# HanielUlises/GCN-GrabCut

Measured on AMD Instinct MI355X. Metric: images/sec end-to-end mask (DUTS-shape batch), higher is better.
Workload: dtype f32

## Files before the change

### gcn-grabcut_amd/csrc/ggc_maxflow.hip

```cpp
#include "ggc_gc.h"
#include "ggc_mf_sweep.h"
#include "ggc_mf_push.h"
#include <algorithm>
#include <chrono>
#include <cstdlib>
#include <vector>

namespace ggc {

constexpr int RT = MF_RT;
constexpr int PT_W = MF_PT_W, PT_H = MF_PT_H;
constexpr int PT_N = PT_W * PT_H;
constexpr int PUSH_GRID = 1024, RELAX_GRID = 1024, ASYNC_GRID = 128;

__global__ void __launch_bounds__(256) k_mf_zero3(int32_t* __restrict__ a, size_t na, int32_t* __restrict__ b, size_t nb, int32_t* __restrict__ c, size_t nc) {
    const size_t i = (size_t)blockIdx.x * 256 + threadIdx.x;
    if (i < na) a[i] = 0;
    else if (i < na + nb) b[i - na] = 0;
    else if (i < na + nb + nc) c[i - na - nb] = 0;
}
void mf_zero3(hipStream_t st, int32_t* a, size_t na, int32_t* b, size_t nb, int32_t* c, size_t nc) {
    const size_t n = na + nb + nc;
    if (n) hipLaunchKernelGGL(k_mf_zero3, dim3(cdiv(n, 256)), dim3(256), 0, st, a, na, b, nb, c, nc);
}

__device__ __forceinline__ void aq_zero(unsigned long long* __restrict__ ring, int32_t* __restrict__ q, int cap) {
    const size_t n_thr = (size_t)gridDim.x * gridDim.y * blockDim.x;
    const size_t i0 = ((size_t)blockIdx.y * gridDim.x + blockIdx.x) * blockDim.x + threadIdx.x;
    for (size_t i = i0; i < (size_t)cap; i += n_thr) ring[i] = 0ull;
    if (i0 < (size_t)AQ_WORDS) q[i0] = 0;
}

constexpr int OUT_CAP = 1024;
struct OutList { int n, base; int buf[OUT_CAP]; };
__device__ __forceinline__ void push_tile_l(int tile, int32_t* __restrict__ flag, OutList& L, int32_t* __restrict__ list,
                                            int32_t* __restrict__ count) {
    if (ldg(&flag[tile]) == 0 && atomicExch(&flag[tile], 1) == 0) {
        const int i = atomicAdd(&L.n, 1);
        if (i < OUT_CAP) L.buf[i] = tile;
        else list[atomicAdd(count, 1)] = tile;
    }
}
__device__ __forceinline__ void flush_tiles(OutList& L, int32_t* __restrict__ list, int32_t* __restrict__ count) {
    __syncthreads();
    const int n = min(L.n, OUT_CAP);
    if (threadIdx.x == 0 && n > 0) L.base = atomicAdd(count, n);
    __syncthreads();
    for (int i = threadIdx.x; i < n; i += blockDim.x) list[L.base + i] = L.buf[i];
}

__global__ void __launch_bounds__(256) k_mf_rinit(GcDims d, MfTiles tl, const int32_t* __restrict__ open_list,
                                                  const int32_t* __restrict__ snk, int32_t* __restrict__ dist,
                                                  int32_t* __restrict__ list, int32_t* __restrict__ flag, int32_t* __restrict__ flag2,
                                                  int32_t* __restrict__ count, int32_t* __restrict__ active, int32_t* __restrict__ scan,
                                                  unsigned long long* __restrict__ ring, int32_t* __restrict__ q, int cap) {
    constexpr int T = MF_RT;
    __shared__ OutList outl;
    if (threadIdx.x == 0) outl.n = 0;
    aq_zero(ring, q, cap);
    if (blockIdx.x == 0 && threadIdx.x == 0) active[open_list[blockIdx.y]] = 0;
    if (blockIdx.x == 0 && blockIdx.y == 0 && threadIdx.x < 8 && (threadIdx.x == 0 || threadIdx.x >= 4)) scan[threadIdx.x] = 0;
    __syncthreads();
    const int tiles_per_image = tl.rt_x * tl.rt_y;
    const int tr = blockIdx.x * 4 + (threadIdx.x >> 6), lane = threadIdx.x & 63;
    if (tr < tiles_per_image) {
        const int b = open_list[blockIdx.y];
        const int ty0 = (tr / tl.rt_x) * T, tx0 = (tr % tl.rt_x) * T;
        const int lx = lane & 31, h = lane >> 5;
        const size_t base = (size_t)b * d.P;
        int sv[16];
#pragma unroll
        for (int r = 0; r < 16; ++r) sv[r] = snk[base + (size_t)min(ty0 + 16 * h + r, d.H - 1) * d.W + min(tx0 + lx, d.W - 1)];
        bool open_px = false;
#pragma unroll
        for (int r = 0; r < 16; ++r) {
            const int y = ty0 + 16 * h + r, x = tx0 + lx;
            if (x < d.W && y < d.H) {
                dist[base + (size_t)y * d.W + x] = sv[r] > 0 ? 1 : DINF;
                open_px |= sv[r] <= 0;
            }
        }
        const bool listed = __any(open_px);
        if (lane == 0) {
            const int tile = b * tiles_per_image + tr;
            flag[tile] = listed ? 1 : 0;
            flag2[tile] = 0;
            if (listed) {
                const int i = atomicAdd(&outl.n, 1);
                if (i < OUT_CAP) outl.buf[i] = tile; else list[atomicAdd(count, 1)] = tile;
            }
        }
    }
    flush_tiles(outl, list, count);
}

template <bool PROF>
__global__ void __launch_bounds__(256) k_mf_relax_wave(GcDims d, MfTiles tl, int phase, long long* __restrict__ prof, uint8_t* __restrict__ rmask,
                                                       int32_t* __restrict__ dirty, const int32_t* __restrict__ rc, int32_t* __restrict__ dist, int32_t* __restrict__ counters,
                                                       const int32_t* __restrict__ list_in, int32_t* __restrict__ list_out,
                                                       int32_t* __restrict__ flag_in, int32_t* __restrict__ flag_out) {
    __shared__ RelaxWaveLds lds[4];
    __shared__ OutList outl;
    if (threadIdx.x == 0) outl.n = 0;
    __syncthreads();
    const int wv = threadIdx.x >> 6;
    const int n_in = counters[phase % 3];
    int32_t* n_out = counters + (phase + 1) % 3;
    if (blockIdx.x == 0 && threadIdx.x == 0) counters[(phase + 2) % 3] = 0;
    const int tiles_per_image = tl.rt_x * tl.rt_y;
    const int G = gridDim.x * 4;
    MfRelaxClocks<PROF> ck;
    int tile_nx = blockIdx.x * 4 + wv < n_in ? list_in[blockIdx.x * 4 + wv] : 0;
    for (int t = blockIdx.x * 4 + wv; t < n_in; t += G) {
        int lane = threadIdx.x & 63;
        asm volatile("" : "+v"(lane));
        ck.begin();
        const int tile = __builtin_amdgcn_readfirstlane(tile_nx);
        tile_nx = t + G < n_in ? list_in[t + G] : 0;
        const int nbm = mf_relax_visit<false, PROF, GGC_MF_RELAX_BFS != 0>(d, tl, tile, lane, lds[wv], rmask, dirty, rc, dist, flag_in, ck);
        const int b = tile / tiles_per_image, tr = tile % tiles_per_image;
        const int tyi = tr / tl.rt_x, txi = tr % tl.rt_x;
        if (lane < 9 && (nbm >> lane) & 1) {
            const int ty = tyi + lane / 3 - 1, tx = txi + lane % 3 - 1;
            if (ty >= 0 && ty < tl.rt_y && tx >= 0 && tx < tl.rt_x)
                push_tile_l(b * tiles_per_image + ty * tl.rt_x + tx, flag_out, outl, list_out, n_out);
        }
        mf_wave_sync();
        ck.end();
    }
    if (PROF && (threadIdx.x & 63) == 0 && ck.sum[3]) {
        unsigned long long* q = reinterpret_cast<unsigned long long*>(prof) + (64 + (blockIdx.x & 63)) * 8;
        for (int k = 0; k < 7; ++k) atomicAdd(&q[k], (unsigned long long)ck.sum[k]);
    }
    flush_tiles(outl, list_out, n_out);
}

#ifndef GGC_MF_PUSH_WAVE
#define GGC_MF_PUSH_WAVE 1
#endif
constexpr int PUSH_WAVE_GRID_DIV = 2;
template <bool PROF>
__global__ void __launch_bounds__(256) k_mf_pr_wave(GcDims d, MfTiles tl, int phase, int inner, long long* __restrict__ prof,
                                                    int32_t* __restrict__ rc, int32_t* __restrict__ ex,
                                                    int32_t* __restrict__ snk, int32_t* __restrict__ dist, uint8_t* __restrict__ rmask,
                                                    int32_t* __restrict__ dirty, int32_t* __restrict__ counters, const int32_t* __restrict__ list_in,
                                                    int32_t* __restrict__ list_out, int32_t* __restrict__ flag_in,
                                                    int32_t* __restrict__ flag_out) {
    __shared__ PushTileLds<PT_H> lds[4];
    __shared__ OutList outl;
    if (threadIdx.x == 0) outl.n = 0;
    __syncthreads();
    const int wv = threadIdx.x >> 6;
    const int n_in = counters[phase % 3];
    int32_t* n_out = counters + (phase + 1) % 3;
    if (blockIdx.x == 0 && threadIdx.x == 0) counters[(phase + 2) % 3] = 0;
    const int tiles_per_image = tl.pt_x * tl.pt_y;
    const size_t BP = (size_t)d.B * d.P;
    const int G = gridDim.x * 4;
    long long pv[4] = {0, 0, 0, 0}, p_all = 0, p_n = 0;
    int tile_nx = blockIdx.x * 4 + wv < n_in ? list_in[blockIdx.x * 4 + wv] : 0;
    for (int t = blockIdx.x * 4 + wv; t < n_in; t += G) {
        int lane = threadIdx.x & 63;
        asm volatile("" : "+v"(lane));
        const long long t_0 = PROF ? wall_clock64() : 0;
        const int tile = __builtin_amdgcn_readfirstlane(tile_nx);
        tile_nx = t + G < n_in ? list_in[t + G] : 0;
        const int b = tile / tiles_per_image, tr = tile % tiles_per_image;
        const int tyi = tr / tl.pt_x, txi = tr % tl.pt_x;
        if (lane == 0) flag_in[tile] = 0;
        const int nbm = push_tile_visit<PT_H, false>(d, tyi, txi, inner, (size_t)b * d.P, BP, rc, ex, snk, dist, rmask, lds[wv], lane, PROF, pv);
        if (lane < 9 && (nbm >> lane) & 1) {
            const int ty = tyi + lane / 3 - 1, tx = txi + lane % 3 - 1;
            if (ty >= 0 && ty < tl.pt_y && tx >= 0 && tx < tl.pt_x) {
                const int nbt = b * tiles_per_image + ty * tl.pt_x + tx;
                if (lane != 4) dirty[nbt] = 1;
                push_tile_l(nbt, flag_out, outl, list_out, n_out);
            }
        }
        mf_wave_sync();
        if (PROF) { p_all += wall_clock64() - t_0; ++p_n; }
    }
    if (PROF && (threadIdx.x & 63) == 0 && p_n) {
        unsigned long long* o = reinterpret_cast<unsigned long long*>(prof) + (192 + (blockIdx.x & 63)) * 8;
        atomicAdd(&o[0], (unsigned long long)pv[0]); atomicAdd(&o[1], (unsigned long long)pv[1]);
        atomicAdd(&o[2], (unsigned long long)(p_all - pv[0] - pv[1]));
        atomicAdd(&o[3], (unsigned long long)p_n); atomicAdd(&o[4], (unsigned long long)pv[2]); atomicAdd(&o[5], (unsigned long long)pv[3]);
    }
    flush_tiles(outl, list_out, n_out);
}

#if !GGC_MF_PUSH_WAVE
__global__ void __launch_bounds__(PT_N) k_mf_pr_list(GcDims d, MfTiles tl, int phase, int inner,
                                                    int32_t* __restrict__ rc, int32_t* __restrict__ ex,
                                                    int32_t* __restrict__ snk, int32_t* __restrict__ dist, uint8_t* __restrict__ rmask,
                                                    int32_t* __restrict__ dirty, int32_t* __restrict__ counters, const int32_t* __restrict__ list_in,
                                                    int32_t* __restrict__ list_out, int32_t* __restrict__ flag_in,
                                                    int32_t* __restrict__ flag_out) {
    __shared__ int s_ex[PT_N];
    __shared__ int s_d[PT_H + 2][PT_W + 2];
    __shared__ int s_rc[8][PT_N];
    __shared__ OutList outl;
    __shared__ int s_nbm;
    const int tid = threadIdx.x, lx = tid & 31;
    if (tid == 0) outl.n = 0;
    const int n_in = counters[phase % 3];
    int32_t* n_out = counters + (phase + 1) % 3;
    if (blockIdx.x == 0 && tid == 0) counters[(phase + 2) % 3] = 0;
    const int tiles_per_image = tl.pt_x * tl.pt_y;
    const size_t BP = (size_t)d.B * d.P;
    constexpr int N_HALO = (PT_H + 2) * (PT_W + 2), HALO_IT = (N_HALO + PT_N - 1) / PT_N;
    struct TileRegs { int e, sk, r[8], hv[HALO_IT]; };
    auto load_tile = [&](int tile, TileRegs& R) {
        const int b = tile / tiles_per_image, tr = tile % tiles_per_image;
        const int tyi = tr / tl.pt_x, txi = tr % tl.pt_x;
        const int x = txi * PT_W + lx;
        const size_t base = (size_t)b * d.P;
        const int y = tyi * PT_H + (tid >> 5);
        const bool in = x < d.W && y < d.H;
        const int p = y * d.W + x;
        R.e = in ? ex[base + p] : 0;
        R.sk = in ? snk[base + p] : 0;
#pragma unroll
        for (int dir = 0; dir < 8; ++dir) R.r[dir] = in ? rc[rc_idx(dir, base + p)] : 0;
#pragma unroll
        for (int k = 0; k < HALO_IT; ++k) {
            const int i = tid + k * PT_N;
            const int gy = tyi * PT_H + i / (PT_W + 2) - 1, gx = txi * PT_W + i % (PT_W + 2) - 1;
            R.hv[k] = (i < N_HALO && gx >= 0 && gx < d.W && gy >= 0 && gy < d.H) ? dist[base + (size_t)gy * d.W + gx] : DINF;
        }
    };
    const int G = gridDim.x;
    int t = blockIdx.x;
    if (t >= n_in) return;
    int tile_next = list_in[t];
    int tile_next2 = t + G < n_in ? list_in[t + G] : 0;
    TileRegs N;
    load_tile(tile_next, N);
    for (; t < n_in; t += G) {
        const int tile = tile_next;
        const int b = tile / tiles_per_image, tr = tile % tiles_per_image;
        const int tyi = tr / tl.pt_x, txi = tr % tl.pt_x;
        const int x = txi * PT_W + lx;
        const size_t base = (size_t)b * d.P;
        __syncthreads();
        const int y = tyi * PT_H + (tid >> 5);
        const bool inb = x < d.W && y < d.H;
        const int pp = y * d.W + x;
        const int e0 = N.e, sk0 = N.sk;
        int sk = sk0, r0[8];
        s_ex[tid] = e0;
#pragma unroll
        for (int dir = 0; dir < 8; ++dir) { r0[dir] = N.r[dir]; s_rc[dir][tid] = r0[dir]; }
#pragma unroll
        for (int k = 0; k < HALO_IT; ++k) {
            const int i = tid + k * PT_N;
            if (i < N_HALO) s_d[i / (PT_W + 2)][i % (PT_W + 2)] = N.hv[k];
        }
        if (t + G < n_in) {
            tile_next = tile_next2;
            tile_next2 = t + 2 * G < n_in ? list_in[t + 2 * G] : 0;
            load_tile(tile_next, N);
        }
        __syncthreads();
        if (tid == 0) { flag_in[tile] = 0; s_nbm = 0; }
        const int d0 = s_d[(tid >> 5) + 1][lx + 1];
        int nbm = 0;
        for (int it = 0; it < inner; ++it) {
            int act = 0;
            if (inb) {
                const int slot = tid, ly = slot >> 5;
                const int e = __hip_atomic_load(&s_ex[slot], __ATOMIC_RELAXED, __HIP_MEMORY_SCOPE_WORKGROUP);
                const int dp = s_d[ly + 1][lx + 1];
                if (e > 0 && dp < d.P) {
                    act = 1;
                    int r[8], hq[8];
#pragma unroll
                    for (int dir = 0; dir < 8; ++dir) {
                        r[dir] = __hip_atomic_load(&s_rc[dir][slot], __ATOMIC_RELAXED, __HIP_MEMORY_SCOPE_WORKGROUP);
                        hq[dir] = s_d[ly + 1 + dir_dy(dir)][lx + 1 + dir_dx(dir)];
                    }
                    int hmin = sk > 0 ? 0 : DINF, best = sk > 0 ? 8 : -1, rb = 0;
#pragma unroll
                    for (int dir = 0; dir < 8; ++dir) {
                        const bool ok = r[dir] > 0 && hq[dir] < hmin;
                        hmin = ok ? hq[dir] : hmin; best = ok ? dir : best; rb = ok ? r[dir] : rb;
                    }
                    if (best >= 0 && dp > hmin) {
                        if (best == 8) {
                            const int dl = min(e, sk);
                            sk -= dl;
                            atomicSub(&s_ex[slot], dl);
                        } else {
                            const int dl = min(e, rb);
                            atomicSub(&s_rc[best][slot], dl);
                            atomicSub(&s_ex[slot], dl);
                            const int bx = dir_dx(best), by = dir_dy(best);
                            const int qlx = lx + bx, qly = ly + by;
                            if (qlx >= 0 && qlx < PT_W && qly >= 0 && qly < PT_H) {
                                const int qt = qly * PT_W + qlx;
                                atomicAdd(&s_rc[best ^ 1][qt], dl);
                                atomicAdd(&s_ex[qt], dl);
                            } else {
                                const int q = pp + by * d.W + bx;
                                atomicAdd(&rc[rc_idx((best ^ 1), base + q)], dl);
                                atomicAdd(&ex[base + q], dl);
                                const int tdy = qly < 0 ? -1 : (qly >= PT_H ? 1 : 0), tdx = qlx < 0 ? -1 : (qlx >= PT_W ? 1 : 0);
                                nbm |= 1 << ((tdy + 1) * 3 + tdx + 1);
                            }
                        }
                    } else {
                        s_d[ly + 1][lx + 1] = (best >= 0 && hmin < DINF) ? hmin + 1 : DINF;
                    }
                }
            }
            if (!__syncthreads_or(act)) break;
        }
        int left = 0;
        if (inb) {
            const int slot = tid, ly = slot >> 5, p = pp;
            const bool ring = lx == 0 || lx == PT_W - 1 || ly == 0 || ly == PT_H - 1;
            const int e1 = s_ex[slot];
            if (e1 != e0) { if (ring) atomicAdd(&ex[base + p], e1 - e0); else ex[base + p] = e1; }
            int m1 = 0, chg = 0;
#pragma unroll
            for (int dir = 0; dir < 8; ++dir) {
                const int r1 = s_rc[dir][slot];
                m1 |= (r1 > 0) ? (1 << dir) : 0;
                if (r1 != r0[dir]) {
                    chg = 1;
                    const bool out = (ly == 0 && dir_dy(dir) < 0) || (ly == PT_H - 1 && dir_dy(dir) > 0) ||
                                     (lx == 0 && dir_dx(dir) < 0) || (lx == PT_W - 1 && dir_dx(dir) > 0);
                    if (out) atomicAdd(&rc[rc_idx(dir, base + p)], r1 - r0[dir]);
                    else rc[rc_idx(dir, base + p)] = r1;
                }
// ... 286 lines not shown
```

### gcn-grabcut_amd/csrc/ggc_maxflow_async.hip

```cpp
#include "ggc_gc.h"
#include "ggc_mf_sweep.h"
#include "ggc_mf_push.h"
#include <algorithm>
#include <cstdlib>

namespace ggc {
namespace {

constexpr int PT_H = MF_PT_H;
constexpr long long AQ_TIMEOUT = 200000000ll;

__device__ __forceinline__ unsigned long long ldg64(const unsigned long long* p) { return __hip_atomic_load(p, __ATOMIC_RELAXED, __HIP_MEMORY_SCOPE_AGENT); }
__device__ __forceinline__ void drain() { asm volatile("s_waitcnt vmcnt(0)" ::: "memory"); }

struct AqInit { const int32_t* list; int n; };

__device__ __forceinline__ int aq_pop(unsigned long long* __restrict__ ring, int32_t* __restrict__ q, int cap, const AqInit& in, int lane,
                                      int32_t* __restrict__ err_flag) {
    int payload = -1;
    if (lane == 0) {
        const unsigned t = (unsigned)atomicAdd(&q[AQ_HEAD], 1);
        if (t < (unsigned)in.n) {
            payload = in.list[t];
        } else {
            const unsigned tr = t - (unsigned)in.n;
            unsigned long long* slot = ring + tr % (unsigned)cap;
            const long long t0 = wall_clock64();
            for (int n = 0;; ++n) {
                const unsigned long long v = ldg64(slot);
                if ((unsigned)(v >> 32) == tr + 1u) { atomicExch(slot, 0ull); payload = (int)(unsigned)v; break; }
                if ((n & 3) == 3) {
                    if (ldg(&q[AQ_DONE]) || ldg(&q[AQ_PENDING]) + in.n == 0) break;
                    if (wall_clock64() - t0 > AQ_TIMEOUT) { if (err_flag) atomicOr(err_flag, 4); atomicExch(&q[AQ_DONE], 1); break; }
                }
                __builtin_amdgcn_s_sleep(4);
            }
        }
    }
    return __builtin_amdgcn_readfirstlane(payload);
}
__device__ __forceinline__ void aq_push(unsigned long long* __restrict__ ring, int32_t* __restrict__ q, int cap, int payload,
                                        int32_t* __restrict__ err_flag) {
    atomicAdd(&q[AQ_PENDING], 1);
    const unsigned t = (unsigned)atomicAdd(&q[AQ_TAIL], 1);
    unsigned long long* slot = ring + t % (unsigned)cap;
    const unsigned long long e = ((unsigned long long)(t + 1u) << 32) | (unsigned)payload;
    const long long t0 = wall_clock64();
    while (atomicCAS(slot, 0ull, e) != 0ull) {
        if (wall_clock64() - t0 > AQ_TIMEOUT) { if (err_flag) atomicOr(err_flag, 4); atomicExch(&q[AQ_DONE], 1); break; }
        __builtin_amdgcn_s_sleep(2);
    }
}
__device__ __forceinline__ void aq_finish(int32_t* __restrict__ q, const AqInit& in) {
    if (atomicSub(&q[AQ_PENDING], 1) + in.n == 1) atomicExch(&q[AQ_DONE], 1);
}

#ifndef GGC_MF_RELAX_ASYNC_BFS
#define GGC_MF_RELAX_ASYNC_BFS 1
#endif
template <bool PROF>
__global__ void __launch_bounds__(256) k_mf_relax_async(GcDims d, MfTiles tl, uint8_t* __restrict__ rmask, int32_t* __restrict__ dirty,
                                                        const int32_t* __restrict__ rc, int32_t* __restrict__ dist, int32_t* __restrict__ flag,
                                                        const int32_t* __restrict__ count, const int32_t* __restrict__ list,
                                                        unsigned long long* __restrict__ ring, int32_t* __restrict__ q, int cap,
                                                        int32_t* __restrict__ err_flag, long long* __restrict__ prof) {
    __shared__ RelaxWaveLds lds[4];
    RelaxWaveLds& S = lds[threadIdx.x >> 6];
    const int tiles_per_image = tl.rt_x * tl.rt_y;
    const AqInit in{list, min(*count, cap)};
    MfRelaxClocks<PROF> ck;
    int tile = -1;
    for (;;) {
        int lane = threadIdx.x & 63;
        asm volatile("" : "+v"(lane));
        if (tile < 0) {
            tile = aq_pop(ring, q, cap, in, lane, err_flag);
            if (tile < 0) break;
            if (lane == 0) atomicExch(&flag[tile], 0);
            drain();
        }
        ck.begin();
        const int nbm = mf_relax_visit<true, PROF, GGC_MF_RELAX_ASYNC_BFS != 0>(d, tl, tile, lane, S, rmask, dirty, rc, dist, flag, ck);
        drain();
        const int b = tile / tiles_per_image, tr = tile % tiles_per_image;
        const int tyi = tr / tl.rt_x, txi = tr % tl.rt_x;
        int nb = -1;
        if (lane < 9 && (nbm >> lane) & 1) {
            const int ty = tyi + lane / 3 - 1, tx = txi + lane % 3 - 1;
            if (ty >= 0 && ty < tl.rt_y && tx >= 0 && tx < tl.rt_x) nb = b * tiles_per_image + ty * tl.rt_x + tx;
        }
        const bool cand = nb >= 0 && ldg(&flag[nb]) == 0;
        const unsigned long long cm = __ballot(cand);
        int next = -1;
        if (cm) {
            const int fl = __ffsll((long long)cm) - 1;
            next = __shfl(nb, fl, 64);
            if (cand && lane != fl && atomicExch(&flag[nb], 1) == 0) aq_push(ring, q, cap, nb, err_flag);
            drain();
        }
        if (next < 0 && lane == 0) aq_finish(q, in);
        tile = next;
        mf_wave_sync();
        ck.end();
    }
    if (PROF && (threadIdx.x & 63) == 0 && ck.sum[3]) {
        unsigned long long* o = reinterpret_cast<unsigned long long*>(prof) + (128 + (blockIdx.x & 63)) * 8;
        for (int k = 0; k < 7; ++k) atomicAdd(&o[k], (unsigned long long)ck.sum[k]);
    }
}

constexpr int ST_Q = 1, ST_BUSY = 2;


template <int TH>
__global__ void __launch_bounds__(64) k_mf_push_async(GcDims d, int bt_x, int bt_y, int pt_y, int inner, int gen_max, int32_t* __restrict__ dirty, int32_t* __restrict__ rc,
                                                      int32_t* __restrict__ ex, int32_t* __restrict__ snk, int32_t* __restrict__ dist,
                                                      uint8_t* __restrict__ rmask, int32_t* __restrict__ st, unsigned long long* __restrict__ ring,
                                                      int32_t* __restrict__ q, int cap, const int32_t* __restrict__ count,
                                                      const int32_t* __restrict__ list, int32_t* __restrict__ err_flag,
                                                      long long* __restrict__ prof) {
    __shared__ PushTileLds<TH> S;
    const int tiles_per_image = bt_x * bt_y;
    const size_t BP = (size_t)d.B * d.P;
    const AqInit in{list, count ? min(*count, cap) : 0};
    const int budget = count ? (int)min((long long)in.n * gen_max + 4096, (long long)0x3fffffff) : ldg(&q[AQ_BUDGET]);
    int tile = -1, gen = 0;
    long long p_wait = 0, p_visit = 0, p_hand = 0, p_n = 0, p_follow = 0, pv[4] = {0, 0, 0, 0};
    const long long t_start = prof ? wall_clock64() : 0;
    for (;;) {
        int lane = threadIdx.x & 63;
        asm volatile("" : "+v"(lane));
        const long long t_0 = prof ? wall_clock64() : 0;
        if (tile < 0) {
            const int payload = aq_pop(ring, q, cap, in, lane, err_flag);
            if (payload < 0) { if (prof) p_wait += wall_clock64() - t_0; break; }
            tile = payload & 0xffffff; gen = payload >> 24;
        } else if (prof) ++p_follow;
        int over = 0;
        if (lane == 0) {
            atomicExch(&st[tile], ST_BUSY);
            over = atomicAdd(&q[AQ_VISITS], 1) >= budget;
            if (over) atomicExch(&q[AQ_DONE], 1);
        }
        drain();
        const long long t_1 = prof ? wall_clock64() : 0;
        const int b = tile / tiles_per_image, tr = tile % tiles_per_image;
        const int tyi = tr / bt_x, txi = tr % bt_x;
        const int nbm = push_tile_visit<TH, true>(d, tyi, txi, inner, (size_t)b * d.P, BP, rc, ex, snk, dist, rmask, S, lane, prof != nullptr, pv);
        drain();
        const long long t_2 = prof ? wall_clock64() : 0;
        const bool left = (nbm >> 4) & 1;
        int nb = -1;
        bool cand = false;
        if (lane == 4) {
            nb = tile;
            const int old = atomicExch(&st[tile], left ? ST_Q : 0);
            if (left) cand = true;
            else if (old & ST_Q) cand = (atomicOr(&st[tile], ST_Q) & (ST_Q | ST_BUSY)) == 0;
        } else if (lane < 9 && (nbm >> lane) & 1) {
            const int ty = tyi + lane / 3 - 1, tx = txi + lane % 3 - 1;
            if (ty >= 0 && ty < bt_y && tx >= 0 && tx < bt_x) {
                nb = b * tiles_per_image + ty * bt_x + tx;
                for (int k = 0; k < TH / PT_H; ++k)
                    if (ty * (TH / PT_H) + k < pt_y) atomicOr(&dirty[(size_t)b * bt_x * pt_y + (size_t)(ty * (TH / PT_H) + k) * bt_x + tx], 1);
                cand = (atomicOr(&st[nb], ST_Q) & (ST_Q | ST_BUSY)) == 0;
            }
        }
        if (gen + 1 >= gen_max) cand = false;
        const unsigned long long cm = __ballot(cand);
        int next = -1;
        if (cm) {
            const int fl = __ffsll((long long)cm) - 1;
            next = __shfl(nb, fl, 64);
            if (cand && lane != fl) aq_push(ring, q, cap, ((gen + 1) << 24) | nb, err_flag);
            drain();
        }
        if (next < 0 && lane == 0) aq_finish(q, in);
        tile = next; gen = gen + 1;
        mf_wave_sync();
        if (prof) { p_wait += t_1 - t_0; p_visit += t_2 - t_1; p_hand += wall_clock64() - t_2; ++p_n; }
    }
    if (prof && (threadIdx.x & 63) == 0) {
        unsigned long long* o = reinterpret_cast<unsigned long long*>(prof) + (blockIdx.x & 63) * 8;
        atomicAdd(&o[0], (unsigned long long)p_wait); atomicAdd(&o[1], (unsigned long long)p_visit); atomicAdd(&o[2], (unsigned long long)p_hand);
        atomicAdd(&o[3], (unsigned long long)p_n); atomicAdd(&o[4], (unsigned long long)p_follow);
        atomicAdd(&o[5], (unsigned long long)(wall_clock64() - t_start)); atomicAdd(&o[6], 1ull);
        unsigned long long* o2 = o + 64 * 8;
        atomicAdd(&o2[0], (unsigned long long)pv[0]); atomicAdd(&o2[1], (unsigned long long)pv[1]); atomicAdd(&o2[2], (unsigned long long)pv[2]);
    }
}

__global__ void __launch_bounds__(256) k_aq_fill_big(const int32_t* __restrict__ count, const int32_t* __restrict__ list, int pt_x, int pt_y,
                                                     int th, int bt_x, int bt_y, int32_t* __restrict__ st,
                                                     unsigned long long* __restrict__ ring, int32_t* __restrict__ q, int budget_per_item) {
    const int i = blockIdx.x * blockDim.x + threadIdx.x;
    const int n = *count;
    if (i == 0) q[AQ_BUDGET] = (int)min((long long)n * budget_per_item + 4096, (long long)0x3fffffff);
    if (i >= n) return;
    const int t = list[i], b = t / (pt_x * pt_y), tr = t % (pt_x * pt_y);
    const int big = b * bt_x * bt_y + ((tr / pt_x) * PT_H / th) * bt_x + tr % pt_x;
    if (atomicOr(&st[big], ST_Q) == 0) {
        const int slot = atomicAdd(&q[AQ_TAIL], 1);
        atomicAdd(&q[AQ_PENDING], 1);
        ring[slot] = (((unsigned long long)(unsigned)(slot + 1)) << 32) | (unsigned)big;
    }
}

}

int maxflow_relax_async(ggc_ctx* ctx, hipStream_t st, const GcDims& d, const MfTiles& tl, uint8_t* rmask, int32_t* dirty, const int32_t* rc, int32_t* dist,
                        const int32_t* count, const int32_t* list, int32_t* flag, unsigned long long* ring, int32_t* q, int cap,
                        int grid, int32_t* err_flag, long long* prof) {
    if (prof)
        hipLaunchKernelGGL(k_mf_relax_async<true>, dim3(grid), dim3(256), 0, st, d, tl, rmask, dirty, rc, dist, flag, count, list, ring, q, cap, err_flag, prof);
    else
        hipLaunchKernelGGL(k_mf_relax_async<false>, dim3(grid), dim3(256), 0, st, d, tl, rmask, dirty, rc, dist, flag, count, list, ring, q, cap, err_flag, prof);
    GGC_LAUNCH_CHECK(ctx);
    return GGC_OK;
}

int maxflow_push_async_tile(int th) { return th >= 32 ? 32 : (th >= 16 ? 16 : 8); }

int maxflow_push_async(ggc_ctx* ctx, hipStream_t st, const GcDims& d, const MfTiles& tl, int th, int inner, int gen_max, int32_t* rc,
                       int32_t* ex, int32_t* snk, int32_t* dist, uint8_t* rmask, int32_t* dirty, const int32_t* count, const int32_t* list, int n_list_max, int32_t* state,
                       unsigned long long* ring, int32_t* q, int waves, int32_t* err_flag, long long* prof) {
    th = maxflow_push_async_tile(th);
    const int bt_x = tl.pt_x, bt_y = cdiv(d.H, th), cap = bt_x * bt_y * d.B;
    gen_max = std::min(gen_max, 127);
    if (th == 8) {
        hipLaunchKernelGGL(k_mf_push_async<8>, dim3(waves), dim3(64), 0, st, d, bt_x, bt_y, tl.pt_y, inner, gen_max, dirty, rc, ex, snk, dist, rmask, state, ring, q, cap,
                           count, list, err_flag, prof);
        GGC_LAUNCH_CHECK(ctx);
        return GGC_OK;
    }
    const int32_t* no_list = nullptr;
    mf_zero3(st, reinterpret_cast<int32_t*>(ring), (size_t)cap * 2, q, AQ_WORDS, state, (size_t)cap);
    hipLaunchKernelGGL(k_aq_fill_big, dim3(cdiv(n_list_max, 256)), dim3(256), 0, st, count, list, tl.pt_x, tl.pt_y, th, bt_x, bt_y, state, ring, q,
                       gen_max);
    if (th == 32)
        hipLaunchKernelGGL(k_mf_push_async<32>, dim3(waves), dim3(64), 0, st, d, bt_x, bt_y, tl.pt_y, inner, gen_max, dirty, rc, ex, snk, dist, rmask, state, ring, q, cap,
                           no_list, no_list, err_flag, prof);
    else
        hipLaunchKernelGGL(k_mf_push_async<16>, dim3(waves), dim3(64), 0, st, d, bt_x, bt_y, tl.pt_y, inner, gen_max, dirty, rc, ex, snk, dist, rmask, state, ring, q, cap,
                           no_list, no_list, err_flag, prof);
    GGC_LAUNCH_CHECK(ctx);
    return GGC_OK;
}

}
```

### gcn-grabcut_amd/csrc/ggc_mf_push.h

```cpp
#pragma once
#include "ggc_gc.h"
#include "ggc_mf_sweep.h"

namespace ggc {

template <int TH>
struct PushTileLds {
    int ex[32 * TH]; int sk[32 * TH]; int d[TH + 2][34]; int rc[8][32 * TH];
    uint32_t mask[32]; unsigned short list[64];
};

template <bool ASYNC>
__device__ __forceinline__ int mf_push_ld(const int32_t* p) { return ASYNC ? ldg(p) : *p; }

template <int TH, bool ASYNC>
__device__ int push_tile_visit(const GcDims& d, int tyi, int txi, int inner, size_t base, size_t BP,
                               int32_t* __restrict__ rc, int32_t* __restrict__ ex, int32_t* __restrict__ snk,
                               int32_t* __restrict__ dist, uint8_t* __restrict__ rmask, PushTileLds<TH>& S, int lane,
                               bool prof, long long (&pv)[4]) {
    constexpr int NPX = TH / 2, HALO = (TH + 2) * 34, HALO_IT = (HALO + 63) / 64;
    const long long tv0 = prof ? wall_clock64() : 0;
    const int lx = lane & 31, r0 = lane >> 5;
    const int x = txi * 32 + lx;
    int e0[NPX], sk0[NPX], r0v[NPX][8];
#pragma unroll
    for (int j = 0; j < NPX; ++j) {
        const int y = tyi * TH + r0 + 2 * j;
        const int pc = min(y, d.H - 1) * d.W + min(x, d.W - 1);
        e0[j] = mf_push_ld<ASYNC>(ex + base + pc);
        sk0[j] = mf_push_ld<ASYNC>(snk + base + pc);
#pragma unroll
        for (int dir = 0; dir < 8; ++dir) r0v[j][dir] = mf_push_ld<ASYNC>(rc + rc_idx(dir, base + pc));
    }
    int* sd = &S.d[0][0];
    int hv[HALO_IT];
#pragma unroll
    for (int k = 0; k < HALO_IT; ++k) {
        const int i = min(lane + k * 64, HALO - 1);
        const int gy = tyi * TH + i / 34 - 1, gx = txi * 32 + i % 34 - 1;
        hv[k] = mf_push_ld<ASYNC>(dist + base + (size_t)min(max(gy, 0), d.H - 1) * d.W + min(max(gx, 0), d.W - 1));
    }
#pragma unroll
    for (int k = 0; k < HALO_IT; ++k) {
        const int i = lane + k * 64;
        const int gy = tyi * TH + i / 34 - 1, gx = txi * 32 + i % 34 - 1;
        if (i < HALO) sd[i] = (gx >= 0 && gx < d.W && gy >= 0 && gy < d.H) ? hv[k] : DINF;
    }
    if (lane < 32) S.mask[lane] = 0u;
    mf_wave_sync();
#pragma unroll
    for (int j = 0; j < NPX; ++j) {
        const int slot = lane + 64 * j, ly = r0 + 2 * j;
        const bool inb = x < d.W && tyi * TH + ly < d.H;
        if (!inb) { e0[j] = 0; sk0[j] = 0; }
        S.ex[slot] = e0[j];
        S.sk[slot] = sk0[j];
#pragma unroll
        for (int dir = 0; dir < 8; ++dir) {
            if (!inb) r0v[j][dir] = 0;
            S.rc[dir][slot] = r0v[j][dir];
        }
        const bool a = e0[j] > 0 && S.d[ly + 1][lx + 1] < d.P;
        const unsigned long long m = __ballot(a);
        if (lane == 0) { S.mask[2 * j] = (uint32_t)m; S.mask[2 * j + 1] = (uint32_t)(m >> 32); }
    }
    mf_wave_sync();
    int nbm = 0;
    const long long tv1 = prof ? wall_clock64() : 0;
    int n_sw = 0, n_deal = 0;
    int cur = -1;
    auto deal = [&]() {
        uint32_t w = 0u;
        int off = 0, n_act = 0;
#pragma unroll
        for (int r = 0; r < TH; ++r) {
            const uint32_t wr = S.mask[r];
            const int cr = __popc(wr);
            w = r == lane ? wr : w;
            off += r < lane ? cr : 0;
            n_act += cr;
        }
        mf_wave_sync();
        while (w && off < 64) { const int bit = __ffs(w) - 1; S.list[off++] = (unsigned short)(lane * 32 + bit); w &= w - 1; }
        if (lane < TH) S.mask[lane] = w;
        mf_wave_sync();
        cur = lane < n_act ? (int)S.list[lane] : -1;
    };
    deal();
    for (int it = 0; it < inner; ++it) {
        uint32_t sp = 0u;
#pragma unroll
        for (int r = 0; r < TH; ++r) sp |= S.mask[r];
        int carry = -1, spill = -1;
        if (cur >= 0) {
            const int slot = cur, ly = slot >> 5, plx = slot & 31;
            const int e = atomicExch(&S.ex[slot], 0);
            const int dp = S.d[ly + 1][plx + 1];
            const int sk = S.sk[slot];
            int r[8], hq[8];
#pragma unroll
            for (int dir = 0; dir < 8; ++dir) {
                r[dir] = __hip_atomic_load(&S.rc[dir][slot], __ATOMIC_RELAXED, __HIP_MEMORY_SCOPE_WORKGROUP);
                hq[dir] = S.d[ly + 1 + dir_dy(dir)][plx + 1 + dir_dx(dir)];
            }
            if (e <= 0) {
            } else if (dp >= d.P) {
                atomicAdd(&S.ex[slot], e);
            } else {
                int hmin = sk > 0 ? 0 : DINF, best = sk > 0 ? 8 : -1, rb = 0;
#pragma unroll
                for (int dir = 0; dir < 8; ++dir) {
                    const bool ok = r[dir] > 0 && hq[dir] < hmin;
                    hmin = ok ? hq[dir] : hmin; best = ok ? dir : best; rb = ok ? r[dir] : rb;
                }
                if (best >= 0 && dp > hmin) {
                    if (best == 8) {
                        const int dl = min(e, sk);
                        S.sk[slot] = sk - dl;
                        if (e - dl > 0) { atomicAdd(&S.ex[slot], e - dl); carry = slot; }
                    } else {
                        const int dl = min(e, rb), rem = e - dl;
                        atomicSub(&S.rc[best][slot], dl);
                        if (rem > 0) atomicAdd(&S.ex[slot], rem);
                        const int qlx = plx + ((0x62 >> best) & 1) - ((0x91 >> best) & 1), qly = ly + ((0xa8 >> best) & 1) - ((0x54 >> best) & 1);
                        if (qlx >= 0 && qlx < 32 && qly >= 0 && qly < TH) {
                            const int qt = qly * 32 + qlx;
                            atomicAdd(&S.rc[best ^ 1][qt], dl);
                            atomicAdd(&S.ex[qt], dl);
                            carry = qt;
                            spill = rem > 0 ? slot : -1;
                        } else {
                            const int gy = tyi * TH + qly, gx = txi * 32 + qlx;
                            const size_t qg = base + (size_t)gy * d.W + gx;
                            atomicAdd(&rc[rc_idx((best ^ 1), qg)], dl);
                            atomicAdd(&ex[qg], dl);
                            const int tdy = qly < 0 ? -1 : (qly >= TH ? 1 : 0), tdx = qlx < 0 ? -1 : (qlx >= 32 ? 1 : 0);
                            nbm |= 1 << ((tdy + 1) * 3 + tdx + 1);
                            carry = rem > 0 ? slot : -1;
                        }
                    }
                } else {
                    const int nd = (best >= 0 && hmin < DINF) ? hmin + 1 : DINF;
                    S.d[ly + 1][plx + 1] = nd;
                    atomicAdd(&S.ex[slot], e);
                    carry = nd >= d.P ? -1 : slot;
                }
            }
        }
        sp = __builtin_amdgcn_readfirstlane(sp);
        if (sp == 0u && !__any(cur >= 0)) break;
        ++n_sw;
        if (sp == 0u) {
            const unsigned long long rem_m = __ballot(spill >= 0);
            if (rem_m) {
                const unsigned long long idle_m = __ballot(carry < 0);
                const int n_rem = __popcll(rem_m), n_idle = __popcll(idle_m);
                const int k_rem = (int)__builtin_amdgcn_mbcnt_hi((uint32_t)(rem_m >> 32), __builtin_amdgcn_mbcnt_lo((uint32_t)rem_m, 0u));
                const int k_idle = (int)__builtin_amdgcn_mbcnt_hi((uint32_t)(idle_m >> 32), __builtin_amdgcn_mbcnt_lo((uint32_t)idle_m, 0u));
                if (spill >= 0) {
                    if (k_rem < n_idle) S.list[k_rem] = (unsigned short)spill;
                    else atomicOr(&S.mask[spill >> 5], 1u << (spill & 31));
                }
                mf_wave_sync();
                if (carry < 0 && k_idle < n_rem) carry = (int)S.list[k_idle];
            }
            cur = carry;
            mf_wave_sync();
        } else {
            if (carry >= 0) atomicOr(&S.mask[carry >> 5], 1u << (carry & 31));
            if (spill >= 0) atomicOr(&S.mask[spill >> 5], 1u << (spill & 31));
            mf_wave_sync();
            deal();
            if (!ASYNC) ++n_deal;
        }
    }
    const long long tv2 = prof ? wall_clock64() : 0;
    if (prof) { pv[0] += tv1 - tv0; pv[1] += tv2 - tv1; pv[2] += n_sw; }
    if (!ASYNC && prof) pv[3] += n_deal;
    int left = 0;
#pragma unroll
    for (int j = 0; j < NPX; ++j) {
        const int slot = lane + 64 * j, ly = r0 + 2 * j;
        const int y = tyi * TH + ly;
        const bool inb = x < d.W && y < d.H;
        const size_t p = base + (size_t)min(y, d.H - 1) * d.W + min(x, d.W - 1);
        const int e1 = S.ex[slot], sk1 = S.sk[slot], d1 = S.d[ly + 1][lx + 1];
        int r1[8];
#pragma unroll
        for (int dir = 0; dir < 8; ++dir) r1[dir] = S.rc[dir][slot];
        if (!inb) continue;
        if (ASYNC) {
            if (e1 != e0[j]) atomicAdd(&ex[p], e1 - e0[j]);
            int m1 = 0, chg = 0;
#pragma unroll
            for (int dir = 0; dir < 8; ++dir) {
                m1 |= (r1[dir] > 0) ? (1 << dir) : 0;
                if (r1[dir] != r0v[j][dir]) { chg = 1; atomicAdd(&rc[rc_idx(dir, p)], r1[dir] - r0v[j][dir]); }
            }
            if (chg) {
                uint32_t* w = reinterpret_cast<uint32_t*>(rmask + (p & ~(size_t)3));
                const int sh = 8 * (int)(p & 3);
                atomicAnd(w, ~(0xffu << sh));
                atomicOr(w, (uint32_t)m1 << sh);
            }
            if (sk1 != sk0[j]) atomicExch(&snk[p], sk1);
        } else {
            const bool ring = lx == 0 || lx == 31 || ly == 0 || ly == TH - 1;
            if (e1 != e0[j]) { if (ring) atomicAdd(&ex[p], e1 - e0[j]); else ex[p] = e1; }
            int m1 = 0, chg = 0;
#pragma unroll
            for (int dir = 0; dir < 8; ++dir) {
                m1 |= (r1[dir] > 0) ? (1 << dir) : 0;
                if (r1[dir] != r0v[j][dir]) {
                    chg = 1;
                    const bool out = (ly == 0 && dir_dy(dir) < 0) || (ly == TH - 1 && dir_dy(dir) > 0) ||
                                     (lx == 0 && dir_dx(dir) < 0) || (lx == 31 && dir_dx(dir) > 0);
                    if (out) atomicAdd(&rc[rc_idx(dir, p)], r1[dir] - r0v[j][dir]);
                    else rc[rc_idx(dir, p)] = r1[dir];
                }
            }
            if (chg) rmask[p] = (uint8_t)m1;
            if (sk1 != sk0[j]) snk[p] = sk1;
        }
        left |= (e1 > 0 && d1 < d.P) ? 1 : 0;
    }
#pragma unroll
    for (int k = 0; k < HALO_IT; ++k) {
        const int i = lane + k * 64;
        const int hy = i / 34, hx = i % 34;
        if (i < HALO && hy >= 1 && hy <= TH && hx >= 1 && hx <= 32) {
            const int gy = tyi * TH + hy - 1, gx = txi * 32 + hx - 1;
            if (gx < d.W && gy < d.H && sd[i] != hv[k]) {
                if (ASYNC) atomicExch(&dist[base + (size_t)gy * d.W + gx], sd[i]);
                else dist[base + (size_t)gy * d.W + gx] = sd[i];
            }
        }
    }
    if (__any(left)) nbm |= 1 << 4;
    return mf_wave_or(nbm);
}

}
```

Before: 4376.

## Write back only touched pixels and overlap tile handover with push writeback

```diff
diff --git a/gcn-grabcut_amd/csrc/ggc_maxflow.hip b/gcn-grabcut_amd/csrc/ggc_maxflow.hip
--- a/gcn-grabcut_amd/csrc/ggc_maxflow.hip
+++ b/gcn-grabcut_amd/csrc/ggc_maxflow.hip
@@ -159,27 +159,41 @@
     const int G = gridDim.x * 4;
     long long pv[4] = {0, 0, 0, 0}, p_all = 0, p_n = 0;
     int tile_nx = blockIdx.x * 4 + wv < n_in ? list_in[blockIdx.x * 4 + wv] : 0;
+    int tile_s = __builtin_amdgcn_readfirstlane(tile_nx);
+    int got = 1, got_tile = 0;
+    auto take = [&]() {
+        if (got == 0) {
+            const int i = atomicAdd(&outl.n, 1);
+            if (i < OUT_CAP) outl.buf[i] = got_tile;
+            else list_out[atomicAdd(n_out, 1)] = got_tile;
+        }
+        got = 1;
+    };
     for (int t = blockIdx.x * 4 + wv; t < n_in; t += G) {
         int lane = threadIdx.x & 63;
         asm volatile("" : "+v"(lane));
         const long long t_0 = PROF ? wall_clock64() : 0;
-        const int tile = __builtin_amdgcn_readfirstlane(tile_nx);
+        const int tile = tile_s;
         tile_nx = t + G < n_in ? list_in[t + G] : 0;
         const int b = tile / tiles_per_image, tr = tile % tiles_per_image;
         const int tyi = tr / tl.pt_x, txi = tr % tl.pt_x;
         if (lane == 0) flag_in[tile] = 0;
-        const int nbm = push_tile_visit<PT_H, false>(d, tyi, txi, inner, (size_t)b * d.P, BP, rc, ex, snk, dist, rmask, lds[wv], lane, PROF, pv);
-        if (lane < 9 && (nbm >> lane) & 1) {
-            const int ty = tyi + lane / 3 - 1, tx = txi + lane % 3 - 1;
-            if (ty >= 0 && ty < tl.pt_y && tx >= 0 && tx < tl.pt_x) {
-                const int nbt = b * tiles_per_image + ty * tl.pt_x + tx;
+        const int nty = tyi + lane / 3 - 1, ntx = txi + lane % 3 - 1;
+        const bool nb_ok = lane < 9 && nty >= 0 && nty < tl.pt_y && ntx >= 0 && ntx < tl.pt_x;
+        const int nbt = nb_ok ? b * tiles_per_image + nty * tl.pt_x + ntx : tile;
+        const int f_pre = ldg(&flag_out[nbt]);
+        push_tile_visit<PT_H, false>(d, tyi, txi, inner, (size_t)b * d.P, BP, rc, ex, snk, dist, rmask, lds[wv], lane, PROF, pv, take,
+                                     [&](int nbm) {
+            tile_s = __builtin_amdgcn_readfirstlane(tile_nx);
+            if (nb_ok && (nbm >> lane) & 1) {
                 if (lane != 4) dirty[nbt] = 1;
-                push_tile_l(nbt, flag_out, outl, list_out, n_out);
+                if (f_pre == 0) { got = atomicExch(&flag_out[nbt], 1); got_tile = nbt; }
             }
-        }
+        });
         mf_wave_sync();
         if (PROF) { p_all += wall_clock64() - t_0; ++p_n; }
     }
+    take();
     if (PROF && (threadIdx.x & 63) == 0 && p_n) {
         unsigned long long* o = reinterpret_cast<unsigned long long*>(prof) + (192 + (blockIdx.x & 63)) * 8;
         atomicAdd(&o[0], (unsigned long long)pv[0]); atomicAdd(&o[1], (unsigned long long)pv[1]);
diff --git a/gcn-grabcut_amd/csrc/ggc_maxflow_async.hip b/gcn-grabcut_amd/csrc/ggc_maxflow_async.hip
--- a/gcn-grabcut_amd/csrc/ggc_maxflow_async.hip
+++ b/gcn-grabcut_amd/csrc/ggc_maxflow_async.hip
@@ -146,7 +146,7 @@
         const long long t_1 = prof ? wall_clock64() : 0;
         const int b = tile / tiles_per_image, tr = tile % tiles_per_image;
         const int tyi = tr / bt_x, txi = tr % bt_x;
-        const int nbm = push_tile_visit<TH, true>(d, tyi, txi, inner, (size_t)b * d.P, BP, rc, ex, snk, dist, rmask, S, lane, prof != nullptr, pv);
+        const int nbm = push_tile_visit<TH, true>(d, tyi, txi, inner, (size_t)b * d.P, BP, rc, ex, snk, dist, rmask, S, lane, prof != nullptr, pv, []() {}, [](int) {});
         drain();
         const long long t_2 = prof ? wall_clock64() : 0;
         const bool left = (nbm >> 4) & 1;
diff --git a/gcn-grabcut_amd/csrc/ggc_mf_push.h b/gcn-grabcut_amd/csrc/ggc_mf_push.h
--- a/gcn-grabcut_amd/csrc/ggc_mf_push.h
+++ b/gcn-grabcut_amd/csrc/ggc_mf_push.h
@@ -4,20 +4,27 @@
 
 namespace ggc {
 
+#ifndef GGC_MF_PUSH_WB_TOUCHED
+#define GGC_MF_PUSH_WB_TOUCHED 1
+#endif
 template <int TH>
 struct PushTileLds {
     int ex[32 * TH]; int sk[32 * TH]; int d[TH + 2][34]; int rc[8][32 * TH];
     uint32_t mask[32]; unsigned short list[64];
+#if GGC_MF_PUSH_WB_TOUCHED
+    uint32_t touch[32];
+#endif
 };
 
 template <bool ASYNC>
 __device__ __forceinline__ int mf_push_ld(const int32_t* p) { return ASYNC ? ldg(p) : *p; }
 
-template <int TH, bool ASYNC>
+template <int TH, bool ASYNC, class LoadsIssued, class HandOver>
 __device__ int push_tile_visit(const GcDims& d, int tyi, int txi, int inner, size_t base, size_t BP,
                                int32_t* __restrict__ rc, int32_t* __restrict__ ex, int32_t* __restrict__ snk,
                                int32_t* __restrict__ dist, uint8_t* __restrict__ rmask, PushTileLds<TH>& S, int lane,
-                               bool prof, long long (&pv)[4]) {
+                               bool prof, long long (&pv)[4], LoadsIssued&& loads_issued, HandOver&& handover) {
+    constexpr bool WBT = GGC_MF_PUSH_WB_TOUCHED != 0 && !ASYNC;
     constexpr int NPX = TH / 2, HALO = (TH + 2) * 34, HALO_IT = (HALO + 63) / 64;
     const long long tv0 = prof ? wall_clock64() : 0;
     const int lx = lane & 31, r0 = lane >> 5;
@@ -40,6 +47,8 @@
         const int gy = tyi * TH + i / 34 - 1, gx = txi * 32 + i % 34 - 1;
         hv[k] = mf_push_ld<ASYNC>(dist + base + (size_t)min(max(gy, 0), d.H - 1) * d.W + min(max(gx, 0), d.W - 1));
     }
+    if constexpr (WBT) __builtin_amdgcn_sched_barrier(0);
+    loads_issued();
 #pragma unroll
     for (int k = 0; k < HALO_IT; ++k) {
         const int i = lane + k * 64;
@@ -47,6 +56,9 @@
         if (i < HALO) sd[i] = (gx >= 0 && gx < d.W && gy >= 0 && gy < d.H) ? hv[k] : DINF;
     }
     if (lane < 32) S.mask[lane] = 0u;
+#if GGC_MF_PUSH_WB_TOUCHED
+    if (WBT && lane < 32) S.touch[lane] = 0u;
+#endif
     mf_wave_sync();
 #pragma unroll
     for (int j = 0; j < NPX; ++j) {
@@ -65,7 +77,13 @@
         if (lane == 0) { S.mask[2 * j] = (uint32_t)m; S.mask[2 * j + 1] = (uint32_t)(m >> 32); }
     }
     mf_wave_sync();
+    if constexpr (WBT) __builtin_amdgcn_s_waitcnt(0x0f70);
     int nbm = 0;
+    auto mark = [&](int slot) {
+#if GGC_MF_PUSH_WB_TOUCHED
+        if constexpr (WBT) atomicOr(&S.touch[slot >> 5], 1u << (slot & 31));
+#endif
+    };
     const long long tv1 = prof ? wall_clock64() : 0;
     int n_sw = 0, n_deal = 0;
     int cur = -1;
@@ -117,16 +135,19 @@
                     if (best == 8) {
                         const int dl = min(e, sk);
                         S.sk[slot] = sk - dl;
+                        mark(slot);
                         if (e - dl > 0) { atomicAdd(&S.ex[slot], e - dl); carry = slot; }
                     } else {
                         const int dl = min(e, rb), rem = e - dl;
                         atomicSub(&S.rc[best][slot], dl);
+                        mark(slot);
                         if (rem > 0) atomicAdd(&S.ex[slot], rem);
                         const int qlx = plx + ((0x62 >> best) & 1) - ((0x91 >> best) & 1), qly = ly + ((0xa8 >> best) & 1) - ((0x54 >> best) & 1);
                         if (qlx >= 0 && qlx < 32 && qly >= 0 && qly < TH) {
                             const int qt = qly * 32 + qlx;
                             atomicAdd(&S.rc[best ^ 1][qt], dl);
                             atomicAdd(&S.ex[qt], dl);
+                            mark(qt);
                             carry = qt;
                             spill = rem > 0 ? slot : -1;
                         } else {
@@ -134,6 +155,7 @@
                             const size_t qg = base + (size_t)gy * d.W + gx;
                             atomicAdd(&rc[rc_idx((best ^ 1), qg)], dl);
                             atomicAdd(&ex[qg], dl);
+                            if constexpr (WBT) atomicAdd(&rc[rc_idx(best, base + (size_t)(tyi * TH + ly) * d.W + txi * 32 + plx)], -dl);
                             const int tdy = qly < 0 ? -1 : (qly >= TH ? 1 : 0), tdx = qlx < 0 ? -1 : (qlx >= 32 ? 1 : 0);
                             nbm |= 1 << ((tdy + 1) * 3 + tdx + 1);
                             carry = rem > 0 ? slot : -1;
@@ -177,67 +199,144 @@
     const long long tv2 = prof ? wall_clock64() : 0;
     if (prof) { pv[0] += tv1 - tv0; pv[1] += tv2 - tv1; pv[2] += n_sw; }
     if (!ASYNC && prof) pv[3] += n_deal;
+    auto store_labels = [&]() {
+#pragma unroll
+        for (int k = 0; k < HALO_IT; ++k) {
+            const int i = lane + k * 64;
+            const int hy = i / 34, hx = i % 34;
+            if (i < HALO && hy >= 1 && hy <= TH && hx >= 1 && hx <= 32) {
+                const int gy = tyi * TH + hy - 1, gx = txi * 32 + hx - 1;
+                if (gx < d.W && gy < d.H && sd[i] != hv[k]) {
+                    if (ASYNC) atomicExch(&dist[base + (size_t)gy * d.W + gx], sd[i]);
+                    else dist[base + (size_t)gy * d.W + gx] = sd[i];
+                }
+            }
+        }
+    };
     int left = 0;
-#pragma unroll
-    for (int j = 0; j < NPX; ++j) {
-        const int slot = lane + 64 * j, ly = r0 + 2 * j;
-        const int y = tyi * TH + ly;
-        const bool inb = x < d.W && y < d.H;
-        const size_t p = base + (size_t)min(y, d.H - 1) * d.W + min(x, d.W - 1);
-        const int e1 = S.ex[slot], sk1 = S.sk[slot], d1 = S.d[ly + 1][lx + 1];
-        int r1[8];
-#pragma unroll
-        for (int dir = 0; dir < 8; ++dir) r1[dir] = S.rc[dir][slot];
-        if (!inb) continue;
-        if (ASYNC) {
-            if (e1 != e0[j]) atomicAdd(&ex[p], e1 - e0[j]);
-            int m1 = 0, chg = 0;
-#pragma unroll
-            for (int dir = 0; dir < 8; ++dir) {
-                m1 |= (r1[dir] > 0) ? (1 << dir) : 0;
-                if (r1[dir] != r0v[j][dir]) { chg = 1; atomicAdd(&rc[rc_idx(dir, p)], r1[dir] - r0v[j][dir]); }
-            }
-            if (chg) {
-                uint32_t* w = reinterpret_cast<uint32_t*>(rmask + (p & ~(size_t)3));
-                const int sh = 8 * (int)(p & 3);
-                atomicAnd(w, ~(0xffu << sh));
-                atomicOr(w, (uint32_t)m1 << sh);
-            }
-            if (sk1 != sk0[j]) atomicExch(&snk[p], sk1);
-        } else {
-            const bool ring = lx == 0 || lx == 31 || ly == 0 || ly == TH - 1;
-            if (e1 != e0[j]) { if (ring) atomicAdd(&ex[p], e1 - e0[j]); else ex[p] = e1; }
-            int m1 = 0, chg = 0;
-#pragma unroll
-            for (int dir = 0; dir < 8; ++dir) {
-                m1 |= (r1[dir] > 0) ? (1 << dir) : 0;
-                if (r1[dir] != r0v[j][dir]) {
-                    chg = 1;
-                    const bool out = (ly == 0 && dir_dy(dir) < 0) || (ly == TH - 1 && dir_dy(dir) > 0) ||
-                                     (lx == 0 && dir_dx(dir) < 0) || (lx == 31 && dir_dx(dir) > 0);
-                    if (out) atomicAdd(&rc[rc_idx(dir, p)], r1[dir] - r0v[j][dir]);
-                    else rc[rc_idx(dir, p)] = r1[dir];
-                }
-            }
-            if (chg) rmask[p] = (uint8_t)m1;
-            if (sk1 != sk0[j]) snk[p] = sk1;
-        }
-        left |= (e1 > 0 && d1 < d.P) ? 1 : 0;
-    }
-#pragma unroll
-    for (int k = 0; k < HALO_IT; ++k) {
-        const int i = lane + k * 64;
-        const int hy = i / 34, hx = i % 34;
-        if (i < HALO && hy >= 1 && hy <= TH && hx >= 1 && hx <= 32) {
-            const int gy = tyi * TH + hy - 1, gx = txi * 32 + hx - 1;
-            if (gx < d.W && gy < d.H && sd[i] != hv[k]) {
-                if (ASYNC) atomicExch(&dist[base + (size_t)gy * d.W + gx], sd[i]);
-                else dist[base + (size_t)gy * d.W + gx] = sd[i];
-            }
-        }
-    }
-    if (__any(left)) nbm |= 1 << 4;
-    return mf_wave_or(nbm);
+    if constexpr (WBT) {
+        store_labels();
+        int e1v[NPX];
+#pragma unroll
+        for (int j = 0; j < NPX; ++j) {
+            const int slot = lane + 64 * j, ly = r0 + 2 * j;
+            e1v[j] = S.ex[slot];
+            left |= (e1v[j] > 0 && S.d[ly + 1][lx + 1] < d.P) ? 1 : 0;
+        }
+        int nb_all = __any(left) ? 1 << 4 : 0;
+#pragma unroll
+        for (int k = 0; k < 9; ++k)
+            if (k != 4) nb_all |= __any((nbm >> k) & 1) ? 1 << k : 0;
+        nbm = nb_all;
+        handover(nbm);
+#pragma unroll
+        for (int j = 0; j < NPX; ++j) {
+            const int ly = r0 + 2 * j, y = tyi * TH + ly;
+            if (x < d.W && y < d.H && e1v[j] != e0[j]) {
+                const size_t p = base + (size_t)y * d.W + x;
+                const bool ring = lx == 0 || lx == 31 || ly == 0 || ly == TH - 1;
+                if (ring) atomicAdd(&ex[p], e1v[j] - e0[j]); else ex[p] = e1v[j];
+            }
+        }
+        for (;;) {
+            uint32_t w = 0u;
+            int off = 0, n_t = 0;
+#pragma unroll
+            for (int r = 0; r < TH; ++r) {
+                const uint32_t wr = S.touch[r];
+                const int cr = __popc(wr);
+                w = r == lane ? wr : w;
+                off += r < lane ? cr : 0;
+                n_t += cr;
+            }
+            n_t = __builtin_amdgcn_readfirstlane(n_t);
+            if (n_t == 0) break;
+            mf_wave_sync();
+            while (w && off < 64) { const int bit = __ffs(w) - 1; S.list[off++] = (unsigned short)(lane * 32 + bit); w &= w - 1; }
+            if (lane < TH) S.touch[lane] = w;
+            mf_wave_sync();
+            if (lane < n_t) {
+                const int slot = (int)S.list[lane], ly = slot >> 5, plx = slot & 31;
+                const int gy = tyi * TH + ly, gx = txi * 32 + plx;
+                int r[8];
+#pragma unroll
+                for (int dir = 0; dir < 8; ++dir) r[dir] = S.rc[dir][slot];
+                const int sk = S.sk[slot];
+                if (gx < d.W && gy < d.H) {
+                    const size_t p = base + (size_t)gy * d.W + gx;
+                    int m1 = 0;
+#pragma unroll
+                    for (int dir = 0; dir < 8; ++dir) m1 |= (r[dir] > 0) ? (1 << dir) : 0;
+                    const int outm = (ly == 0 ? 0x54 : 0) | (ly == TH - 1 ? 0xa8 : 0) | (plx == 0 ? 0x91 : 0) | (plx == 31 ? 0x62 : 0);
+                    if (outm == 0) {
+                        int4* q = reinterpret_cast<int4*>(rc + rc_idx(0, p));
+                        q[0] = make_int4(r[0], r[1], r[2], r[3]);
+                        q[1] = make_int4(r[4], r[5], r[6], r[7]);
+                    } else {
+#pragma unroll
+                        for (int dir = 0; dir < 8; ++dir)
+                            if (!((outm >> dir) & 1)) rc[rc_idx(dir, p)] = r[dir];
+                    }
+                    rmask[p] = (uint8_t)m1;
+                    snk[p] = sk;
+                }
+            }
+            if (n_t <= 64) break;
+            mf_wave_sync();
+        }
+    } else {
+#pragma unroll
+        for (int j = 0; j < NPX; ++j) {
+            const int slot = lane + 64 * j, ly = r0 + 2 * j;
+            const int y = tyi * TH + ly;
+            const bool inb = x < d.W && y < d.H;
+            const size_t p = base + (size_t)min(y, d.H - 1) * d.W + min(x, d.W - 1);
+            const int e1 = S.ex[slot], sk1 = S.sk[slot], d1 = S.d[ly + 1][lx + 1];
+            int r1[8];
+#pragma unroll
+            for (int dir = 0; dir < 8; ++dir) r1[dir] = S.rc[dir][slot];
+            if (!inb) continue;
+            if (ASYNC) {
+                if (e1 != e0[j]) atomicAdd(&ex[p], e1 - e0[j]);
+                int m1 = 0, chg = 0;
+#pragma unroll
+                for (int dir = 0; dir < 8; ++dir) {
+                    m1 |= (r1[dir] > 0) ? (1 << dir) : 0;
+                    if (r1[dir] != r0v[j][dir]) { chg = 1; atomicAdd(&rc[rc_idx(dir, p)], r1[dir] - r0v[j][dir]); }
+                }
+                if (chg) {
+                    uint32_t* w = reinterpret_cast<uint32_t*>(rmask + (p & ~(size_t)3));
+                    const int sh = 8 * (int)(p & 3);
+                    atomicAnd(w, ~(0xffu << sh));
+                    atomicOr(w, (uint32_t)m1 << sh);
+                }
+                if (sk1 != sk0[j]) atomicExch(&snk[p], sk1);
+            } else {
+                const bool ring = lx == 0 || lx == 31 || ly == 0 || ly == TH - 1;
+                if (e1 != e0[j]) { if (ring) atomicAdd(&ex[p], e1 - e0[j]); else ex[p] = e1; }
+                int m1 = 0, chg = 0;
+#pragma unroll
+                for (int dir = 0; dir < 8; ++dir) {
+                    m1 |= (r1[dir] > 0) ? (1 << dir) : 0;
+                    if (r1[dir] != r0v[j][dir]) {
+                        chg = 1;
+                        const bool out = (ly == 0 && dir_dy(dir) < 0) || (ly == TH - 1 && dir_dy(dir) > 0) ||
+                                         (lx == 0 && dir_dx(dir) < 0) || (lx == 31 && dir_dx(dir) > 0);
+                        if (out) atomicAdd(&rc[rc_idx(dir, p)], r1[dir] - r0v[j][dir]);
+                        else rc[rc_idx(dir, p)] = r1[dir];
+                    }
+                }
+                if (chg) rmask[p] = (uint8_t)m1;
+                if (sk1 != sk0[j]) snk[p] = sk1;
+            }
+            left |= (e1 > 0 && d1 < d.P) ? 1 : 0;
+        }
+        if (__any(left)) nbm |= 1 << 4;
+        nbm = mf_wave_or(nbm);
+    }
+    if constexpr (!WBT) store_labels();
+    if constexpr (!WBT) handover(nbm);
+    return nbm;
 }
 
 }
```

Result: no change. 4396, median of 4 (+0.4%).
